# swami1995/diff-qp-mpc

Hardware: AMD Instinct MI355X
Metric: QPs/sec (fwd+bwd), batch=4096 n=3 m=3 T=5 (higher is better)
Workload: dtype f64; 1 GPU; random dense QP family R (SURVEY 8d), configs[0] shape at the BASELINE metric batch: B=4096/GPU nz=30 nineq=30 neq=15; global_batch=4096, n_state=3, n_ctrl=3, T=5, parallelism=batch-shard x1, termination=batch (the reference's batch-coupled rule, parity-safe)

## Files before the change

diff-qp-mpc_amd/_build.py:

```python
import os
import shutil
import subprocess

HERE = os.path.dirname(os.path.abspath(__file__))
CSRC = os.path.join(HERE, "csrc")
SO = os.path.join(CSRC, "libdqp_hip.so")
ARCH = "gfx950"

R16_SIZES = [
    (30, 30, 15),
    (20, 10, 15),
    (15, 10, 10),
    (25, 10, 20),
    (10, 5, 3), (12, 8, 0),
]
R16N_SIZES = [s for s in R16_SIZES if s[2] > 0] + [
    (40, 20, 30),
    (35, 10, 30),
]

RIC_HOST_PARTS = [
    [(15, 1), (14, 2), (13, 3), (11, 5)], [(10, 6), (9, 7), (8, 8)],
    [(31, 1)], [(30, 2)], [(29, 3)], [(28, 4)], [(27, 5)], [(26, 6)], [(25, 7)],
]
# ... 8 lines not shown
def hipcc():
    for c in (os.environ.get("HIPCC"), shutil.which("hipcc"), "/opt/rocm/bin/hipcc"):
        if c and os.path.exists(c):
            return c
    raise RuntimeError("hipcc not found (set HIPCC=/path/to/hipcc)")


def _deps():
    d = [os.path.join(CSRC, f) for f in os.listdir(CSRC) if f.endswith((".hip", ".h", ".hpp"))]
    d.append(os.path.join(os.path.dirname(HERE), "include", "dqp.h"))
    d.append(os.path.abspath(__file__))
    return d


def needs_build():
    if not os.path.exists(SO):
        return True
    t = os.path.getmtime(SO)
    return any(os.path.getmtime(d) > t for d in _deps() if os.path.exists(d))


def _jobs():
    cc = hipcc()
    jobs = []
    variants = [("r16f", "dqp_r16.hip", R16_SIZES, []), ("r16b", "dqp_r16.hip", R16_SIZES, ["-DDQP_R16_BWD"]),
                ("r16n", "dqp_r16n.hip", R16N_SIZES, []), ("r16nb", "dqp_r16n.hip", R16N_SIZES, ["-DDQP_R16_BWD"])]
    for tag, src, sizes, extra in variants:
        for n, m, e in sorted(sizes, key=lambda t: -t[0] * t[1]):
            obj = os.path.join(CSRC, "dqp_%s_%d_%d_%d.o" % (tag, n, m, e))
            jobs.append((obj, [cc] + FLAGS + extra + ["-DDQP_R16_N=%d" % n, "-DDQP_R16_M=%d" % m,
                                                      "-DDQP_R16_E=%d" % e, "-c",
                                                      os.path.join(CSRC, src), "-o", obj]))
    for src in PLAIN_SOURCES:
# ... 11 lines not shown
            if "ric" in name and "pad" not in name:
                return 10 ** 5
            return 10 ** 9 if "pdipm" in name else 1
        n, mm, e = m
        w = n * n * (n + mm)
        return w * (4 if "_r16n_" in name else (1 if "_r16nb_" in name else 2))
    jobs.sort(key=cost, reverse=True)
    lst = lambda sizes: " ".join("X(%d,%d,%d)" % s for s in sizes)
    obj = os.path.join(CSRC, "dqp_dispatch.o")
    jobs.append((obj, [cc] + FLAGS + ["-DDQP_R16_SIZE_LIST=" + lst(R16_SIZES),
                                      "-DDQP_R16N_SIZE_LIST=" + lst(R16N_SIZES),
                                      "-c", os.path.join(CSRC, "dqp_dispatch.hip"), "-o", obj]))
    return jobs


def _object_current(obj, cmd):
    stamp = obj + ".cmd"
    if not (os.path.exists(obj) and os.path.exists(stamp)):
        return False
    with open(stamp) as f:
        if f.read() != " ".join(cmd):
            return False
    src = cmd[cmd.index("-c") + 1]
    deps = [src]
    dfile = obj[:-2] + ".d"
    if os.path.exists(dfile):
        with open(dfile) as f:
            words = f.read().replace("\\\n", " ").split()
        deps += [w for w in words[1:] if w.startswith((CSRC, os.path.dirname(HERE)))]
    else:
        deps += [os.path.join(os.path.dirname(HERE), "include", "dqp.h")]
        deps += [os.path.join(CSRC, f) for f in os.listdir(CSRC) if f.endswith((".h", ".hpp"))]
    t = os.path.getmtime(obj)
    return all(os.path.exists(d) and os.path.getmtime(d) <= t for d in deps)


def build(force=False, verbose=False, max_parallel=None):
    if not force and not needs_build():
        return SO
    jobs = _jobs()
    todo = [j for j in jobs if force or not _object_current(*j)]
    all_jobs, jobs = jobs, todo
    max_parallel = max_parallel or max(1, min(len(jobs), (os.cpu_count() or 2)))
    import time
    pending, running = list(jobs), []
    while pending or running:
        while pending and len(running) < max_parallel:
            obj, cmd = pending.pop(0)
            if verbose:
                print(" ".join(cmd))
            running.append((subprocess.Popen(cmd), cmd))
        still = []
        for pr, cmd in running:
            rc = pr.poll()
            if rc is None:
                still.append((pr, cmd))
            elif rc != 0:
                for other, _ in running:
                    if other.poll() is None:
                        other.kill()
                raise subprocess.CalledProcessError(rc, cmd)
            else:
                with open(cmd[-1] + ".cmd", "w") as f:
                    f.write(" ".join(cmd))
        if len(still) == len(running):
            time.sleep(0.2)
        running = still
    subprocess.check_call([hipcc(), "--offload-arch=" + ARCH, "-shared", "-fPIC", "-o", SO] +
                          [obj for obj, _ in all_jobs])
    return SO


if __name__ == "__main__":
    print(build(force=True, verbose=True))
```

diff-qp-mpc_amd/csrc/dqp_common.h:

```cpp
#ifndef DQP_COMMON_H_
#define DQP_COMMON_H_
#include <hip/hip_runtime.h>
#include <stdint.h>

#include "../../include/dqp.h"
#include "dqp_trace.h"

namespace dqp {

constexpr int WAVE = 64;

struct KParams {
    const double *Q, *p, *G, *h, *A, *b;
    long long sQ, sp, sG, sh, sA, sb;
    double *zhat, *lam, *nu, *slack, *best_resid;
    const double *zin, *lamin, *nuin, *slackin, *gin;
    double *dQ, *dp, *dG, *dh, *dA, *db;
    int32_t *info;
    double *workspace;
    unsigned long long *stamps;
    int B, N, M, E;
    int ldz, ldm, lde, ldt;
    double eps, stallTol;
    int maxIter, notImprovedLim;
    unsigned flags;
    double *hist;
    const int32_t *cap;
    int histIters;
    int dynId, dynT, dynN, dynM;
    double dynDt;
    const double *dynX0;
    const double *mC, *mc, *mF, *mf, *mx0, *mul, *muu;
    double *mdC, *mdc, *mdF, *mdf, *mdx0;
    int mn, mm, mT;
    double *snap;
    const double *histIn;
    const double *extRy;
    int itBegin, itEnd;
};

constexpr int TERM_HDR = 8;

constexpr int TERM_MAXIT = 64;
constexpr int TERM_ACC_BYTES = 3 * 8 + TERM_HDR * 4;

__device__ __forceinline__ void hist_put(const KParams &P, long long qp, int it, double resid, double mu)
{
    double2 *h = reinterpret_cast<double2 *>(P.hist) + (long long)it * P.B + qp;
    *h = make_double2(resid, mu);
}
__device__ __forceinline__ void hist_fill(const KParams &P, long long qp, int iters)
{
    const double nan = __builtin_nan("");
    for (int it = iters; it < P.histIters; ++it)
        reinterpret_cast<double2 *>(P.hist)[(long long)it * P.B + qp] = make_double2(nan, nan);
}
__device__ __forceinline__ void term_zero_acc(const KParams &P)
{
    if (P.hist && blockIdx.x == 0) {
        unsigned *a = reinterpret_cast<unsigned *>(P.hist + (long long)P.B * P.histIters * 2);
        for (int i = threadIdx.x; i < TERM_ACC_BYTES / 4; i += blockDim.x) a[i] = 0u;
    }
}

__device__ __forceinline__ bool term_flagged(const KParams &P, long long qp) { return P.cap[TERM_HDR + qp] >= P.cap[0]; }

size_t term_bytes(int B, int maxIter, int snapDim);
int term_decide(const KParams &P, void *term, void *stream);
int term_local_masks(const KParams &P, void *term, unsigned long long *masks, void *stream);
int term_decide_global(const KParams &P, void *term, const unsigned long long *masks, void *stream);
void term_bind_pass1(KParams &P, void *term, int snapDim);
void term_bind_pass2(KParams &P, void *term);


#ifdef DQP_STAMPS
extern unsigned long long *g_debug_stamps;
#endif
int r16_forward(const KParams &P, void *stream);
int r16_backward(const KParams &P, void *stream);
int r16n_forward(const KParams &P, void *stream);
long long r16n_workspace_doubles(int N, int M, int E);
int r16n_snapshot_doubles(int N, int M, int E);
bool ric_supported(int n_state, int n_ctrl);
long long ric_workspace_doubles(int n_state, int n_ctrl, int T);
int ric_forward(const KParams &P, void *stream);
long long ric_stepped_workspace_doubles(int n_state, int n_ctrl, int T, int B);
int ric_forward_stepped(const KParams &P, void *stream);
int ric_backward(const KParams &P, void *stream);
int ric_snapshot_doubles(int n_state, int n_ctrl, int T);
int ric_finish(const KParams &P, void *stream);
bool ricw_supported(int n_state, int n_ctrl);
long long ricw_workspace_doubles(int n_state, int n_ctrl, int T);
int ricw_forward(const KParams &P, void *stream);
long long ricw_stepped_workspace_doubles(int n_state, int n_ctrl, int T, int B);
int ricw_forward_stepped(const KParams &P, void *stream);
int ricw_backward(const KParams &P, void *stream);
int ricw_snapshot_doubles(int n_state, int n_ctrl, int T);
// ... 40 lines not shown
```

diff-qp-mpc_amd/csrc/dqp_dispatch.hip:

```cpp
#include "dqp_common.h"

#ifndef DQP_R16_SIZE_LIST
#error "DQP_R16_SIZE_LIST not defined (see _build.py)"
#endif
#ifndef DQP_R16N_SIZE_LIST
#define DQP_R16N_SIZE_LIST
#endif

namespace dqp {

#define X(n, m, e)                                                  \
    int r16_forward_##n##_##m##_##e(const KParams &, void *);       \
    int r16_backward_##n##_##m##_##e(const KParams &, void *);
DQP_R16_SIZE_LIST
#undef X
#define X(n, m, e)                                                  \
    int r16n_forward_##n##_##m##_##e(const KParams &, void *);      \
    int r16n_backward_##n##_##m##_##e(const KParams &, void *);
DQP_R16N_SIZE_LIST
#undef X

int r16_forward(const KParams &P, void *stream)
{
#define X(n, m, e) if (P.N == n && P.M == m && P.E == e) return r16_forward_##n##_##m##_##e(P, stream);
    DQP_R16_SIZE_LIST
#undef X
    return 1;
}

int r16_backward(const KParams &P, void *stream)
{
#define X(n, m, e) if (P.N == n && P.M == m && P.E == e) return r16_backward_##n##_##m##_##e(P, stream);
// ... 6 lines not shown
{
#define X(n, m, e) if (P.N == n && P.M == m && P.E == e) return r16n_forward_##n##_##m##_##e(P, stream);
    DQP_R16N_SIZE_LIST
#undef X
    return 1;
}

int r16n_backward(const KParams &P, void *stream)
{
#define X(n, m, e) if (P.N == n && P.M == m && P.E == e) return r16n_backward_##n##_##m##_##e(P, stream);
    DQP_R16N_SIZE_LIST
#undef X
    return 1;
}

long long r16n_workspace_doubles(int N, int M, int E)
{
#define X(n, m, e)                                                                          \
    if (N == n && M == m && E == e)                                                         \
        return (long long)e * (n - e) + (long long)e * (e - 1) / 2 + (long long)n * (n + 1) / 2 + \
               (long long)m * n + (long long)e * e + 5 * e + n + 1;
    DQP_R16N_SIZE_LIST
#undef X
    return 0;
}

int r16n_snapshot_doubles(int N, int M, int E)
{
    return r16n_workspace_doubles(N, M, E) > 0 ? (N - E) + 2 * M + 2 : 0;
}
// ... 3 lines not shown
```

diff-qp-mpc_amd/csrc/dqp_pdipm.hip:

```cpp

#include <hip/hip_runtime.h>
#include <math.h>
#include <stdint.h>

#include "dqp_common.h"
#include "dqp_dyn_models.h"

using namespace dqp;

namespace {

#define WSYNC() __syncthreads()

__device__ __forceinline__ double bcast(double v, int src)
{
    int lo = __double2loint(v), hi = __double2hiint(v);
    lo = __builtin_amdgcn_readlane(lo, src);
    hi = __builtin_amdgcn_readlane(hi, src);
    return __hiloint2double(hi, lo);
}

template <int CTRL> __device__ __forceinline__ double dppd(double v)
{
    return __builtin_amdgcn_update_dpp(v, v, CTRL, 0xf, 0xf, true);
// ... 711 lines not shown
    if (rc != DQP_OK) return rc;
    if (P.B == 0) return DQP_OK;
    if (!Q || !p || !G || !h || !zhat || !lam || !slack) return DQP_ERR_BAD_ARG;
    P.workspace = (double *)workspace;
    if (P.E > 0 && (!A || !b || !nu)) return DQP_ERR_BAD_ARG;
    P.Q = Q; P.p = p; P.G = G; P.h = h; P.A = A; P.b = b;
    P.zhat = zhat; P.lam = lam; P.nu = nu; P.slack = slack;
    P.info = info; P.best_resid = best_resid;
    if (!(P.flags & DQP_FLAG_BATCH_TERMINATION)) return forward_once(P, lds, workspace, stream);
    if (!termination || P.maxIter < 1 || P.maxIter > 64) return DQP_ERR_BAD_ARG;
    P.eps = opts ? opts->eps : 1e-12;
    const bool nullspace = workspace && !(P.flags & (DQP_FLAG_GENERIC_ONLY | DQP_FLAG_NO_NULLSPACE)) && !P.dynId && !is_big(P);
    term_bind_pass1(P, termination, nullspace ? r16n_snapshot_doubles(P.N, P.M, P.E) : 0);
    if ((rc = forward_once(P, lds, workspace, stream)) != DQP_OK) return rc;
    if (P.flags & DQP_FLAG_HISTORY_ONLY) return DQP_OK;
    if ((rc = term_decide(P, termination, stream)) != DQP_OK) return rc;
    term_bind_pass2(P, termination);
    return forward_once(P, lds, workspace, stream);
}

__attribute__((visibility("default"))) int
dqp_term_local_masks(const dqp_dims *dims, const dqp_opts *opts, void *termination, uint64_t *masks, void *stream)
{
    KParams P = {};
    size_t lds = 0;
    int rc = fill_params(dims, opts, P, lds);
    if (rc != DQP_OK) return rc;
    if (!(P.flags & DQP_FLAG_BATCH_TERMINATION) || !termination || !masks || P.maxIter < 1 || P.maxIter > 64)
        return DQP_ERR_BAD_ARG;
    if (P.B == 0) return hipMemsetAsync(masks, 0, 24, (hipStream_t)stream) == hipSuccess ? DQP_OK : DQP_ERR_LAUNCH;
// ... 167 lines not shown
    if (kind == MPC_PAD) {
        R = pad_region(P.workspace + pad_kernel_doubles(P.mn, P.mm, P.mT, P.B, false), P.mn, P.mm, P.mT, P.B);
        rc = pad_pack(md->n_state, P.mn, P.mm, P.mT, P.B, R, C, c, F, f, x0, nullptr, nullptr, nullptr, nullptr, stream);
        if (rc != DQP_OK) return rc;
        P.mC = R.C; P.mc = R.c; P.mF = R.F; P.mf = R.f; P.mx0 = R.x0; P.zhat = R.tau; P.nu = R.nu;
    }
    auto done = [&](int r) {
        if (r != DQP_OK || kind != MPC_PAD) return r;
        return pad_unpack(md->n_state, P.mn, P.mm, P.mT, P.B, R, tau, nu, nullptr, nullptr, nullptr, nullptr, nullptr, stream);
    };
    if (!batch) return done(run(P));
    P.eps = opts ? opts->eps : 1e-12;
    term_bind_pass1(P, termination, mpc_snapshot_doubles(P, kind));
    if ((rc = run(P)) != DQP_OK) return rc;
    if (P.flags & DQP_FLAG_HISTORY_ONLY) return done(DQP_OK);
    if ((rc = term_decide(P, termination, stream)) != DQP_OK) return rc;
    term_bind_pass2(P, termination);
    return done(kind == MPC_R16N ? r16n_forward(P, stream) : ric_finish(P, stream));
}

static int stage_snapshot_doubles(int n, int m, int T)
{
    return stage_supported(n, m) ? T * (2 * n + 5 * m) : 0;
}

static int stepped_params(const dqp_mpc_dims *md, const dqp_opts *opts, KParams &P)
{
    if (!md || md->nbatch < 0 || md->n_state <= 0 || md->n_ctrl <= 0 || md->T < 2 || !md->has_bounds) return DQP_ERR_BAD_ARG;
    int np = md->n_state;
    if (md->n_state_host) {
// ... 158 lines not shown
```

diff-qp-mpc_amd/csrc/dqp_r16_prims.h:

```cpp
#ifndef DQP_R16_PRIMS_H_
#define DQP_R16_PRIMS_H_
#include <hip/hip_runtime.h>
#include <math.h>

#include "dqp_common.h"

namespace dqp {
namespace r16 {

template <int CTRL> __device__ __forceinline__ double dppd(double v)
{
    return __builtin_amdgcn_update_dpp(v, v, CTRL, 0xf, 0xf, true);
}

__device__ __forceinline__ double rb(double v, int k)
{
    switch (k & 15) {
    case 0: return dppd<0x150>(v);   case 1: return dppd<0x151>(v);
    case 2: return dppd<0x152>(v);   case 3: return dppd<0x153>(v);
    case 4: return dppd<0x154>(v);   case 5: return dppd<0x155>(v);
    case 6: return dppd<0x156>(v);   case 7: return dppd<0x157>(v);
    case 8: return dppd<0x158>(v);   case 9: return dppd<0x159>(v);
    case 10: return dppd<0x15a>(v);  case 11: return dppd<0x15b>(v);
    case 12: return dppd<0x15c>(v);  case 13: return dppd<0x15d>(v);
// ... 378 lines not shown
        }
        __syncthreads();
        const double *row = stage + (r < nr ? r : 0) * NC;
#pragma unroll
        for (int j = 0; j < NC; ++j) dst[s][j] = row[j];
        if (16 * s + 15 >= nrows) {
            const double keep = r < nr ? 1.0 : 0.0;
#pragma unroll
            for (int j = 0; j < NC; ++j) dst[s][j] *= keep;
        }
        __syncthreads();
    }
}

template <int S, int NC>
__device__ __forceinline__ void load_rows(const double *src, int nrows, double (&dst)[S][NC], int r)
{
#pragma unroll
    for (int s = 0; s < S; ++s) {
        const int i = r + 16 * s;
        const double *row = src + (i < nrows ? i : nrows - 1) * NC;
        const double keep = i < nrows ? 1.0 : 0.0;
#pragma unroll
        for (int j = 0; j < NC; ++j) dst[s][j] = row[j];
        if (16 * s + 15 >= nrows) {
#pragma unroll
            for (int j = 0; j < NC; ++j) dst[s][j] *= keep;
        }
    }
}

template <class C>
__device__ __forceinline__ void factor_T(double *lds, double (&T)[C::SM][C::M],
                                         const double (&rdiag)[C::SM], const double (&dinv)[C::SM],
                                         double (&rdu)[C::SM], int r)
{
    constexpr int M = C::M, SM = C::SM;
    double *Rp = lds + C::oR;
#pragma unroll
    for (int s = 0; s < SM; ++s) {
        const int i = r + 16 * s;
        double *dst = i < M ? Rp + tri(i) + i : lds + C::oDummy + r;
        *dst = rdiag[s] + dinv[s];
    }
// ... 21 lines not shown
```

diff-qp-mpc_amd/csrc/dqp_r16n.hip:

```cpp

#include "dqp_r16_prims.h"

namespace dqp {
namespace r16n {

using namespace dqp::r16;

template <int N_, int M_, int E_> struct Cfg {
    static constexpr int N = N_, M = M_, E = E_, R = N_ - E_;
    static constexpr int SN = slots(N_), SM = slots(M_), SR = slots(N_ - E_);
    static constexpr int SE = E_ > 0 ? slots(E_) : 1, EC = E_ > 0 ? E_ : 1;
    static constexpr bool PARK = slots(N_) >= 3;
#ifndef DQP_R16N_PARK_WU
#define DQP_R16N_PARK_WU 1
#endif
    static constexpr bool PARKWU = PARK || DQP_R16N_PARK_WU;
#ifndef DQP_R16N_PIN_ALL
#define DQP_R16N_PIN_ALL 1
#endif
    static constexpr bool PIN = PARK || DQP_R16N_PIN_ALL;
#ifndef DQP_R16N_SPLIT_ALL
#define DQP_R16N_SPLIT_ALL 0
#endif
    static constexpr bool SPLIT = PARK || DQP_R16N_SPLIT_ALL;
#ifndef DQP_R16N_EARLY_CTX
#define DQP_R16N_EARLY_CTX 1
#endif
    static constexpr bool EARLY = DQP_R16N_EARLY_CTX;
    static constexpr int tailsz = E_ * (N_ - E_) + E_ * (E_ - 1) / 2;
    static constexpr int oLq = 0;
    static constexpr int oTl = tri(N_);
    static constexpr int oR = oTl;
    static constexpr int shared = tailsz > tri(M_) ? tailsz : tri(M_);
    static constexpr int oCp = oTl + shared;
    static constexpr int oHp = oCp + (N_ - E_);
    static constexpr int oQv = oHp + M_;
    static constexpr int oBw = oQv + N_;
    static constexpr int oBs = oBw + (N_ - E_), oBz = oBs + M_, oBc = oBz + M_;
    static constexpr int oDummy = oBc + 2;
    static constexpr int ldsQP = oDummy + 16;
    static constexpr int ldsQPpad = (ldsQP + 1) & ~1;
#ifndef DQP_R16N_STAGED
#define DQP_R16N_STAGED 0
#endif
    static constexpr bool STAGED = DQP_R16N_STAGED && 16 * N_ <= ldsQP - oTl;
    __host__ __device__ static constexpr int toff(int k) { return k * (N_ - E_) + k * (k - 1) / 2; }
    static constexpr int wTl = 0, wLq = tailsz, wG = wLq + tri(N_), wU = wG + M_ * N_;
    static constexpr int wTau = wU + E_ * E_, wRdu = wTau + E_, wRdq = wRdu + E_;
    static constexpr int wXy = wRdq + N_, wPy = wXy + E_, wW1 = wPy + E_, wDl = wW1 + E_;
    static constexpr int wsQP = wDl + 1;
    static constexpr int snapDim = (N_ - E_) + 2 * M_ + 2;
};

#define DQP_PHASE_FENCE() asm volatile("" ::: "memory")
__device__ __forceinline__ void pin(double &x) { asm volatile("" : "+v"(x) : : "memory"); }
__device__ __forceinline__ const double *relabel(const double *p)
{
    asm volatile("" : "+v"(p));
    return p;
}
// ... 161 lines not shown
}
template <int S, int NC>
__device__ __forceinline__ void mpc_rows_G(const KParams &P, int nrows, double (&dst)[S][NC], int r)
{
    const int n = P.mn, m = P.mm, nt = n + m, half = P.mT * m;
#pragma unroll
    for (int s = 0; s < S; ++s) {
        const int i = r + 16 * s;
        const int k = i < half ? i : i - half;
        const int t = k / m, col = t * nt + n + (k - t * m);
        const double sg = i < half ? 1.0 : -1.0;
#pragma unroll
        for (int c = 0; c < NC; ++c) dst[s][c] = (c == col && i < nrows) ? sg : 0.0;
    }
}
template <int S, int NC>
__device__ __forceinline__ void mpc_rows_A(const KParams &P, long long qp, int nrows, double (&dst)[S][NC], int r)
{
    const int n = P.mn, nt = n + P.mm, T = P.mT;
#pragma unroll
    for (int s = 0; s < S; ++s) {
        const int e = r + 16 * s, ec = e < nrows ? e : nrows - 1;
        const int t = ec / n, j = ec - t * n;
        const bool dynrow = t < T - 1;
        const double *row = P.mF + (((long long)(dynrow ? t : 0) * P.B + qp) * n + j) * nt;
        int tc = 0, jc = 0;
#pragma unroll
        for (int c = 0; c < NC; ++c) {
            const double f = row[jc];
            double v;
            if (dynrow) v = (tc == t) ? f : ((tc == t + 1 && jc == j) ? -1.0 : 0.0);
            else v = (tc == 0 && jc == j) ? 1.0 : 0.0;
            dst[s][c] = e < nrows ? v : 0.0;
            if (++jc == nt) { jc = 0; ++tc; }
        }
    }
}

template <class C>
__device__ __forceinline__ void park_GU(double *ws, const State<C> &st, int r)
{
    constexpr int N = C::N, M = C::M, E = C::E, R = C::R;
#pragma unroll
    for (int s = 0; s < C::SM; ++s) {
// ... 106 lines not shown
            b0[s] = (E > 0 && e < E) ? v : 0.0;
        }
    } else {
#pragma unroll
        for (int s = 0; s < SN; ++s) p0[s] = (r + 16 * s < N) ? P.p[qp * P.sp + r + 16 * s] : 0.0;
#pragma unroll
        for (int s = 0; s < SM; ++s) h0[s] = (r + 16 * s < M) ? P.h[qp * P.sh + r + 16 * s] : 0.0;
#pragma unroll
        for (int s = 0; s < SE; ++s) b0[s] = (E > 0 && r + 16 * s < E) ? P.b[qp * P.sb + r + 16 * s] : 0.0;
    }
    {
        double Lq[SN][N];
        if (mpc) mpc_rows_Q<SN, N>(P, qp, Lq, r);
        else if (C::STAGED) load_rows_staged<SN, N, (N * N) % 2 == 0>(P.Q + qp * P.sQ, N, Lq, r, lds + C::oTl);
        else load_rows<SN, N>(P.Q + qp * P.sQ, N, Lq, r);
        if (!chol_rows<SN, N>(Lq, st.rdq, r)) st.status = DQP_STATUS_Q_NOT_PD;
        tri_store<SN, N>(lds + C::oLq, Lq, r, dummy);
    }
    __syncthreads();
    if (C::EARLY) {
        double *ws = P.workspace + qp * (long long)C::wsQP;
        for (int e = r; e < tri(N); e += 16) ws[C::wLq + e] = lds[C::oLq + e];
#pragma unroll
        for (int s = 0; s < SN; ++s)
            if (r + 16 * s < N) ws[C::wRdq + r + 16 * s] = st.rdq[s];
    }
    __builtin_amdgcn_sched_barrier(0);
    DQP_PHASE_FENCE();
    STAMP(P, 1);

    if (mpc) {
        if (!C::SPLIT) mpc_rows_G<SM, N>(P, M, st.Gh, r);
        if (E > 0) mpc_rows_A<SE, N>(P, qp, E, st.Ah, r);
    } else {
        if (C::STAGED) {
            if (!C::SPLIT) load_rows_staged<SM, N, (M * N) % 2 == 0>(P.G + qp * P.sG, M, st.Gh, r, lds + C::oTl);
            if (E > 0) load_rows_staged<SE, N, (C::EC * N) % 2 == 0>(P.A + qp * P.sA, E, st.Ah, r, lds + C::oTl);
        } else {
            if (!C::SPLIT) load_rows<SM, N>(P.G + qp * P.sG, M, st.Gh, r);
            if (E > 0) load_rows<SE, N>(P.A + qp * P.sA, E, st.Ah, r);
        }
    }
    {
        const double *Lp = lds + C::oLq;
#pragma unroll
        for (int j = 0; j < N; ++j) {
#pragma unroll
            for (int k = 0; k < j; ++k) {
                const double ljk = Lp[tri(j) + k];
                if (!C::SPLIT) {
// ... 313 lines not shown

    {
        if (!C::EARLY) {
            double *ws = P.workspace + qp * (long long)C::wsQP;
            for (int e = r; e < C::tailsz; e += 16) ws[C::wTl + e] = lds[C::oTl + e];
            for (int e = r; e < tri(N); e += 16) ws[C::wLq + e] = lds[C::oLq + e];
            if (!C::PARKWU) park_GU<C>(ws, st, r);
#pragma unroll
            for (int s = 0; s < SN; ++s)
                if (r + 16 * s < N) ws[C::wRdq + r + 16 * s] = st.rdq[s];
        }
    }
    __syncthreads();
    {
        double *Rp = lds + C::oR;
#pragma unroll
        for (int j = 0; j < M; ++j) {
            const int sj = j >> 4, lj = j & 15;
            double acc[SM];
#pragma unroll
            for (int s = 0; s < SM; ++s) acc[s] = 0.0;
#pragma unroll
            for (int c = 0; c < R; ++c) {
                const double gb = rb(st.Gh[sj][c], lj);
#pragma unroll
                for (int s = 0; s < SM; ++s)
                    if (16 * s + 15 >= j) acc[s] = fma(st.Gh[s][c], gb, acc[s]);
            }
#pragma unroll
            for (int s = 0; s < SM; ++s) {
                if (16 * s + 15 < j) continue;
                const int i = r + 16 * s;
                double *dst = (i < M && j <= i) ? Rp + tri(i) + j : dummy;
                *dst = acc[s];
            }
        }
    }
    __syncthreads();
#pragma unroll
    for (int s = 0; s < SM; ++s) {
        const int i = r + 16 * s;
        const double v = (lds + C::oR)[tri(i < M ? i : M - 1) + (i < M ? i : M - 1)];
        st.rdiag[s] = i < M ? v : 0.0;
    }
    __builtin_amdgcn_sched_barrier(0);
    DQP_PHASE_FENCE();
}

template <class C>
// ... 60 lines not shown
        for (int s = 0; s < SN; ++s)
            if (r + 16 * s < N) P.zhat[qp * N + r + 16 * s] = xh[s];
#pragma unroll
        for (int s = 0; s < SM; ++s)
            if (inM[s]) { P.lam[qp * M + r + 16 * s] = bz[s]; P.slack[qp * M + r + 16 * s] = bs[s]; }
        if (E > 0) {
#pragma unroll
            for (int s = 0; s < SE; ++s)
                if (r + 16 * s < E) P.nu[qp * E + r + 16 * s] = yv[s];
        }
        if (r == 0) {
            if (P.info) { P.info[2 * qp] = st.status; P.info[2 * qp + 1] = iters; }
            if (P.best_resid) P.best_resid[qp] = best;
        }
    }
}

template <class C>
__global__ __launch_bounds__(64) void forward_kernel(KParams P)
{
    constexpr int N = C::N, M = C::M, E = C::E, R = C::R;
    constexpr int SN = C::SN, SM = C::SM, SE = C::SE, SR = C::SR;
    extern __shared__ __attribute__((aligned(16))) double sm[];
    const int lane = threadIdx.x, r = lane & 15, qrow = lane >> 4;
    long long qp = (long long)blockIdx.x * 4 + qrow;
    bool live = qp < P.B;
    if (!live) qp = P.B - 1;
    int maxIter = P.maxIter;
    const bool batch = (P.flags & DQP_FLAG_BATCH_TERMINATION) != 0;
    const bool strict = (P.flags & DQP_FLAG_STRICT_GET_STEP) != 0;
    if (P.cap) {
        maxIter = min(maxIter, P.cap[0]);
        live = live && term_flagged(P, qp);
        if (__builtin_amdgcn_ballot_w64(live) == 0) return;
    }
    double *lds = sm + qrow * C::ldsQPpad;
    double *dummy = lds + C::oDummy + r;

    term_zero_acc(P);
    State<C> st;
    STAMP(P, 0);
    setup<C>(P, qp, r, lds, st);
    STAMP(P, 15);

    bool inM[SM], inR[SR];
#pragma unroll
    for (int s = 0; s < SM; ++s) inM[s] = r + 16 * s < M;
#pragma unroll
    for (int s = 0; s < SR; ++s) inR[s] = r + 16 * s < R;

    double T[SM][M], rdu[SM];
    double w[SR], s_[SM], z[SM];
    double cc = 1.0, delta = 0.0;
    {
// ... 24 lines not shown
#pragma unroll
        for (int s = 0; s < SM; ++s) {
            if (ms < 0.0 && inM[s]) s_[s] -= ms - 1.0;
            if (mz < 0.0 && inM[s]) z[s] -= mz - 1.0;
        }
        delta = mz < 0.0 ? 1.0 - mz : 0.0;
        if (r == 0) P.workspace[qp * (long long)C::wsQP + C::wDl] = delta;
    }

    double gz[SR];
    mul_GzT<C>(st, z, gz, r);
    STAMP(P, 6);
    double best = INFINITY, bestc = 1.0;
    bool have_best = false, done = false;
    int nNot = 0, iters = 0;

    for (int it = 0; it < maxIter; ++it) {
        double rw[SR], rz[SM];
        {
            double cp[SR], hp[SM], gw[SM];
            vec_get<SR>(lds + C::oCp, cp, R, r);
            vec_get<SM>(lds + C::oHp, hp, M, r);
            mul_Gz<C>(st, w, gw);
#pragma unroll
            for (int s = 0; s < SR; ++s) rw[s] = inR[s] ? w[s] + cp[s] + gz[s] : 0.0;
#pragma unroll
            for (int s = 0; s < SM; ++s) rz[s] = inM[s] ? gw[s] + s_[s] - hp[s] : 0.0;
        }
        double sz = 0.0, nz2 = 0.0;
#pragma unroll
        for (int s = 0; s < SM; ++s) { sz = fma(s_[s], z[s], sz); nz2 = fma(rz[s], rz[s], nz2); }
        double nx2 = rx_norm2_partial<C>(st, lds, rw, cc * delta, r);
        sz = row_sum(sz); nz2 = row_sum(nz2); nx2 = row_sum(nx2);
        const double mu = fabs(sz * (1.0 / M));
        const double resid = sqrt(nz2) + sqrt(nx2) + M * mu;
        if (!done) {
            iters = it + 1;
            if (!have_best || resid < best) {
                nNot = 0; have_best = true; best = resid; bestc = cc;
                vec_put<SR>(lds + C::oBw, w, R, r, dummy);
                vec_put<SM>(lds + C::oBs, s_, M, r, dummy);
                vec_put<SM>(lds + C::oBz, z, M, r, dummy);
                if (P.snap && live) {
                    double *sp = P.snap + ((long long)it * P.B + qp) * C::snapDim;
#pragma unroll
                    for (int s = 0; s < SR; ++s)
                        if (inR[s]) sp[r + 16 * s] = w[s];
#pragma unroll
                    for (int s = 0; s < SM; ++s)
                        if (inM[s]) { sp[R + r + 16 * s] = s_[s]; sp[R + M + r + 16 * s] = z[s]; }
                    if (r == 0) sp[R + 2 * M] = cc;
                }
            } else {
                nNot += 1;
            }
            if (batch) {
                if (P.hist && r == 0 && live) hist_put(P, qp, it, resid, mu);
                done = !(fabs(resid) < INFINITY);
            } else if ((nNot >= P.notImprovedLim && best < P.stallTol) || best < P.eps || mu > 1e32 ||
                       !(fabs(resid) < INFINITY))
                done = true;
        }
        if (__builtin_amdgcn_ballot_w64(!done) == 0) break;
        if (it == 1) STAMP(P, 9);

        double dza[SM], dsa[SM];
        {
            double gu[SM];
            mul_Gz<C>(st, rw, gu);
#pragma unroll
            for (int s = 0; s < SM; ++s) dza[s] = rz[s] - s_[s] - gu[s];
        }
// ... 39 lines not shown
        lu_solve<SM, M>(T, rdu, dzc, r);
        if (it == 1) STAMP(P, 12);
        tm = 0.0;
#pragma unroll
        for (int s = 0; s < SM; ++s) {
            dz[s] = dza[s] + dzc[s];
            ds[s] = fma(-rsc[s] - dzc[s], dinv[s], dsa[s]);
            tm = fmax(tm, fmax(-dz[s] * rzv[s], -ds[s] * rsv[s]));
        }
        if (strict) {
#pragma unroll
            for (int s = 0; s < SM; ++s) zero_step |= inM[s] && (dz[s] == 0.0 || ds[s] == 0.0);
            if ((__builtin_amdgcn_ballot_w64(zero_step) >> (lane & 48)) & 0xffffull) done = true;
        }
        __builtin_amdgcn_sched_barrier(0);
        double gtd[SR];
        mul_GzT<C>(st, dz, gtd, r);
        alpha = frcp(fmax(row_max(tm) * (1.0 / 0.999), 1.0));
        if (!done) {
#pragma unroll
            for (int s = 0; s < SR; ++s) {
                w[s] = fma(alpha, -rw[s] - gtd[s], w[s]);
                gz[s] = fma(alpha, gtd[s], gz[s]);
            }
#pragma unroll
            for (int s = 0; s < SM; ++s) { s_[s] = fma(alpha, ds[s], s_[s]); z[s] = fma(alpha, dz[s], z[s]); }
            cc *= (1.0 - alpha);
        }
        if (it == 1) STAMP(P, 13);
        if (it == 0) STAMP(P, 8);
    }
    STAMP(P, 7);

    if (P.hist && r == 0 && live) hist_fill(P, qp, iters);
    epilogue<C>(P, qp, r, lds, st, bestc, delta, iters, best, live, true);
    STAMP(P, 14);
}

template <class C>
__device__ __forceinline__ void load_ctx(const KParams &P, long long qp, int r, double *lds, State<C> &st)
{
    constexpr int N = C::N, M = C::M, E = C::E, R = C::R;
    constexpr int SN = C::SN, SM = C::SM, SE = C::SE;
    st.status = DQP_STATUS_OK;
    {
        const double *ws = P.workspace + qp * (long long)C::wsQP;
        for (int e = r; e < C::tailsz; e += 16) lds[C::oTl + e] = ws[C::wTl + e];
        for (int e = r; e < tri(N); e += 16) lds[C::oLq + e] = ws[C::wLq + e];
#pragma unroll
        for (int s = 0; s < SM; ++s) {
// ... 25 lines not shown
            st.rdq[s] = i < N ? v : 0.0;
        }
    }
}

template <class C>
__global__ __launch_bounds__(64) void finish_kernel(KParams P)
{
    constexpr int M = C::M, E = C::E, R = C::R;
    constexpr int SM = C::SM, SE = C::SE, SR = C::SR;
    extern __shared__ __attribute__((aligned(16))) double sm[];
    const int lane = threadIdx.x, r = lane & 15, qrow = lane >> 4;
    long long qp = (long long)blockIdx.x * 4 + qrow;
    bool live = qp < P.B;
    if (!live) qp = P.B - 1;
    live = live && term_flagged(P, qp);
    if (__builtin_amdgcn_ballot_w64(live) == 0) return;
    const int cap = min(P.maxIter, P.cap[0]);
    double *lds = sm + qrow * C::ldsQPpad;
    double *dummy = lds + C::oDummy + r;
    State<C> st;
    load_ctx<C>(P, qp, r, lds, st);
    const double *ws = P.workspace + qp * (long long)C::wsQP;
#pragma unroll
    for (int s = 0; s < SE; ++s) {
        const int k = r + 16 * s, kc = k < E ? k : (E > 0 ? E - 1 : 0);
        const double a = ws[C::wXy + kc], b = ws[C::wPy + kc], c = ws[C::wW1 + kc];
        st.xy[s] = (E > 0 && k < E) ? a : 0.0;
        st.py[s] = (E > 0 && k < E) ? b : 0.0;
        st.w1[s] = (E > 0 && k < E) ? c : 0.0;
    }
    const double delta = ws[C::wDl];
    const double2 *h = reinterpret_cast<const double2 *>(P.histIn) + qp;
// ... 226 lines not shown
}

#if !defined(DQP_R16_N) || !defined(DQP_R16_M) || !defined(DQP_R16_E)
#error "compile with -DDQP_R16_N=.. -DDQP_R16_M=.. -DDQP_R16_E=.."
#endif
#define DQP_CAT2(a, n, m, e) a##n##_##m##_##e
#define DQP_CAT(a, n, m, e) DQP_CAT2(a, n, m, e)

#ifndef DQP_R16_BWD
int DQP_CAT(r16n_forward_, DQP_R16_N, DQP_R16_M, DQP_R16_E)(const KParams &P, void *stream)
{
    using C = r16n::Cfg<DQP_R16_N, DQP_R16_M, DQP_R16_E>;
    if (P.cap && P.snap && P.histIn) return r16n::launch<C>(r16n::finish_kernel<C>, P, stream);
    return r16n::launch<C>(r16n::forward_kernel<C>, P, stream);
}
#else
int DQP_CAT(r16n_backward_, DQP_R16_N, DQP_R16_M, DQP_R16_E)(const KParams &P, void *stream)
{
    using C = r16n::Cfg<DQP_R16_N, DQP_R16_M, DQP_R16_E>;
    return r16n::launch<C>(r16n::backward_kernel<C>, P, stream);
}
#endif

}
```

diff-qp-mpc_amd/csrc/dqp_term.hip:

```cpp
#include "dqp_common.h"

namespace dqp {

namespace {

constexpr int MAXIT = TERM_MAXIT;
struct Acc {
    unsigned long long improved;
    unsigned long long notbelow;
    unsigned long long notabove;
};
static_assert(sizeof(Acc) + TERM_HDR * sizeof(int32_t) == TERM_ACC_BYTES, "layout shared with dqp_common.h");

inline size_t hist_bytes(int B, int maxIter) { return (size_t)B * maxIter * 2 * sizeof(double); }

__device__ __forceinline__ unsigned long long wave_or_u64(unsigned long long v)
{
#pragma unroll
    for (int off = 32; off > 0; off >>= 1) v |= __shfl_xor(v, off, 64);
    return v;
}

__device__ __forceinline__ int rule_stop(unsigned long long ai, unsigned long long anb, unsigned long long ana, int maxIter,
                                         int notImprovedLim)
{
    int nNot = 0;
    for (int it = 0; it < maxIter; ++it) {
        if (it == 0 || ((ai >> it) & 1ull)) nNot = 0;
        else nNot += 1;
        if (nNot == notImprovedLim || !((anb >> it) & 1ull) || !((ana >> it) & 1ull)) return it + 1;
    }
    return maxIter;
}

constexpr int SCAN_CHUNK = 32;
__global__ __launch_bounds__(64) void term_scan_kernel(const double2 *hist, Acc *acc, int32_t *hdr,
                                                       int B, int maxIter, int notImprovedLim, double eps,
                                                       int decide)
{
    const int lane = threadIdx.x;
    const long long qp = (long long)blockIdx.x * blockDim.x + lane;
    const bool live = qp < B;
    unsigned long long imp = 0ull, nb = 0ull, na = 0ull;
    if (live) {
        const double2 *h = hist + qp;
        double best = 0.0;
        int arg = 0;
// ... 62 lines not shown
{
    P.hist = (double *)term;
    P.histIters = P.maxIter;
    P.cap = nullptr;
    P.histIn = nullptr;
    P.snap = snapDim > 0 ? (double *)((char *)term + snap_offset(P.B, P.maxIter)) : nullptr;
}

void term_bind_pass2(KParams &P, void *term)
{
    P.hist = nullptr;
    P.histIn = (const double *)term;
    P.cap = hdr_of(term, P.B, P.maxIter);
}

int term_decide(const KParams &P, void *term, void *stream)
{
    const int blocks = (P.B + 63) / 64;
    DQP_LAUNCH(term_scan_kernel, dim3(blocks), dim3(64), 0, (hipStream_t)stream,
                       (const double2 *)term, acc_of(term, P.B, P.maxIter), hdr_of(term, P.B, P.maxIter),
                       P.B, P.maxIter, P.notImprovedLim, P.eps, 1);
    return hipGetLastError() == hipSuccess ? DQP_OK : DQP_ERR_LAUNCH;
}

int term_local_masks(const KParams &P, void *term, unsigned long long *masks, void *stream)
{
    const int blocks = (P.B + 63) / 64;
    DQP_LAUNCH(term_scan_kernel, dim3(blocks), dim3(64), 0, (hipStream_t)stream,
                       (const double2 *)term, acc_of(term, P.B, P.maxIter), hdr_of(term, P.B, P.maxIter),
                       P.B, P.maxIter, P.notImprovedLim, P.eps, 0);
// ... 15 lines not shown
```

Measured before the change: 16.06 million QPs/sec.

## Fuse termination mask reduction into r16n forward kernel, prefetch tails, group R GEMM

```diff
diff --git a/diff-qp-mpc_amd/_build.py b/diff-qp-mpc_amd/_build.py
--- a/diff-qp-mpc_amd/_build.py
+++ b/diff-qp-mpc_amd/_build.py
@@ -5,6 +5,8 @@
 HERE = os.path.dirname(os.path.abspath(__file__))
 CSRC = os.path.join(HERE, "csrc")
 SO = os.path.join(CSRC, "libdqp_hip.so")
+TERM_SCAN_SO = os.path.join(CSRC, "libdqp_hip_termscan.so")
+TERM_SCAN_SIZES = [(30, 30, 15)]
 ARCH = "gfx950"
 
 R16_SIZES = [
@@ -46,9 +48,9 @@
 
 
 def needs_build():
-    if not os.path.exists(SO):
+    if not os.path.exists(SO) or not os.path.exists(TERM_SCAN_SO):
         return True
-    t = os.path.getmtime(SO)
+    t = min(os.path.getmtime(SO), os.path.getmtime(TERM_SCAN_SO))
     return any(os.path.getmtime(d) > t for d in _deps() if os.path.exists(d))
 
 
@@ -90,6 +92,15 @@
     return jobs
 
 
+def _term_scan_jobs(jobs):
+    out = {}
+    for obj, cmd in jobs:
+        if os.path.basename(obj) in ["dqp_r16n_%d_%d_%d.o" % s for s in TERM_SCAN_SIZES]:
+            o2 = obj[:-2] + ".termscan.o"
+            out[obj] = (o2, cmd[:-1] + [o2, "-DDQP_R16N_TERM_SCAN=1"])
+    return out
+
+
 def _object_current(obj, cmd):
     stamp = obj + ".cmd"
     if not (os.path.exists(obj) and os.path.exists(stamp)):
@@ -115,7 +126,8 @@
     if not force and not needs_build():
         return SO
     jobs = _jobs()
-    todo = [j for j in jobs if force or not _object_current(*j)]
+    variant = _term_scan_jobs(jobs)
+    todo = [j for j in list(variant.values()) + jobs if force or not _object_current(*j)]
     all_jobs, jobs = jobs, todo
     max_parallel = max_parallel or max(1, min(len(jobs), (os.cpu_count() or 2)))
     import time
@@ -137,13 +149,15 @@
                         other.kill()
                 raise subprocess.CalledProcessError(rc, cmd)
             else:
-                with open(cmd[-1] + ".cmd", "w") as f:
+                with open(cmd[cmd.index("-o") + 1] + ".cmd", "w") as f:
                     f.write(" ".join(cmd))
         if len(still) == len(running):
             time.sleep(0.2)
         running = still
     subprocess.check_call([hipcc(), "--offload-arch=" + ARCH, "-shared", "-fPIC", "-o", SO] +
                           [obj for obj, _ in all_jobs])
+    subprocess.check_call([hipcc(), "--offload-arch=" + ARCH, "-shared", "-fPIC", "-o", TERM_SCAN_SO] +
+                          [variant[obj][0] if obj in variant else obj for obj, _ in all_jobs])
     return SO
 
 
diff --git a/diff-qp-mpc_amd/csrc/dqp_common.h b/diff-qp-mpc_amd/csrc/dqp_common.h
--- a/diff-qp-mpc_amd/csrc/dqp_common.h
+++ b/diff-qp-mpc_amd/csrc/dqp_common.h
@@ -35,6 +35,7 @@
     int mn, mm, mT;
     double *snap;
     const double *histIn;
+    const unsigned long long *capMasks;
     const double *extRy;
     int itBegin, itEnd;
 };
@@ -63,6 +64,27 @@
     }
 }
 
+__device__ __forceinline__ void term_zero_acc_agent(const KParams &P)
+{
+    if (P.hist && blockIdx.x == 0) {
+        unsigned *a = reinterpret_cast<unsigned *>(P.hist + (long long)P.B * P.histIters * 2);
+        for (int i = threadIdx.x; i < TERM_ACC_BYTES / 4; i += blockDim.x)
+            __hip_atomic_store(a + i, 0u, __ATOMIC_RELAXED, __HIP_MEMORY_SCOPE_AGENT);
+    }
+}
+
+__device__ __forceinline__ int rule_stop(unsigned long long ai, unsigned long long anb, unsigned long long ana, int maxIter,
+                                         int notImprovedLim)
+{
+    int nNot = 0;
+    for (int it = 0; it < maxIter; ++it) {
+        if (it == 0 || ((ai >> it) & 1ull)) nNot = 0;
+        else nNot += 1;
+        if (nNot == notImprovedLim || !((anb >> it) & 1ull) || !((ana >> it) & 1ull)) return it + 1;
+    }
+    return maxIter;
+}
+
 __device__ __forceinline__ bool term_flagged(const KParams &P, long long qp) { return P.cap[TERM_HDR + qp] >= P.cap[0]; }
 
 size_t term_bytes(int B, int maxIter, int snapDim);
@@ -71,6 +93,7 @@
 int term_decide_global(const KParams &P, void *term, const unsigned long long *masks, void *stream);
 void term_bind_pass1(KParams &P, void *term, int snapDim);
 void term_bind_pass2(KParams &P, void *term);
+void term_bind_pass2_masks(KParams &P, void *term);
 
 
 #ifdef DQP_STAMPS
@@ -81,6 +104,7 @@
 int r16n_forward(const KParams &P, void *stream);
 long long r16n_workspace_doubles(int N, int M, int E);
 int r16n_snapshot_doubles(int N, int M, int E);
+bool r16n_term_in_pass1(int N, int M, int E);
 bool ric_supported(int n_state, int n_ctrl);
 long long ric_workspace_doubles(int n_state, int n_ctrl, int T);
 int ric_forward(const KParams &P, void *stream);
diff --git a/diff-qp-mpc_amd/csrc/dqp_dispatch.hip b/diff-qp-mpc_amd/csrc/dqp_dispatch.hip
--- a/diff-qp-mpc_amd/csrc/dqp_dispatch.hip
+++ b/diff-qp-mpc_amd/csrc/dqp_dispatch.hip
@@ -16,6 +16,7 @@
 #undef X
 #define X(n, m, e)                                                  \
     int r16n_forward_##n##_##m##_##e(const KParams &, void *);      \
+    bool r16n_term_in_pass1_##n##_##m##_##e();                      \
     int r16n_backward_##n##_##m##_##e(const KParams &, void *);
 DQP_R16N_SIZE_LIST
 #undef X
@@ -52,6 +53,14 @@
     return 1;
 }
 
+bool r16n_term_in_pass1(int N, int M, int E)
+{
+#define X(n, m, e) if (N == n && M == m && E == e) return r16n_term_in_pass1_##n##_##m##_##e();
+    DQP_R16N_SIZE_LIST
+#undef X
+    return false;
+}
+
 long long r16n_workspace_doubles(int N, int M, int E)
 {
 #define X(n, m, e)                                                                          \
diff --git a/diff-qp-mpc_amd/csrc/dqp_pdipm.hip b/diff-qp-mpc_amd/csrc/dqp_pdipm.hip
--- a/diff-qp-mpc_amd/csrc/dqp_pdipm.hip
+++ b/diff-qp-mpc_amd/csrc/dqp_pdipm.hip
@@ -749,6 +749,10 @@
     term_bind_pass1(P, termination, nullspace ? r16n_snapshot_doubles(P.N, P.M, P.E) : 0);
     if ((rc = forward_once(P, lds, workspace, stream)) != DQP_OK) return rc;
     if (P.flags & DQP_FLAG_HISTORY_ONLY) return DQP_OK;
+    if (nullspace && r16n_term_in_pass1(P.N, P.M, P.E)) {
+        term_bind_pass2_masks(P, termination);
+        return forward_once(P, lds, workspace, stream);
+    }
     if ((rc = term_decide(P, termination, stream)) != DQP_OK) return rc;
     term_bind_pass2(P, termination);
     return forward_once(P, lds, workspace, stream);
@@ -946,6 +950,10 @@
     term_bind_pass1(P, termination, mpc_snapshot_doubles(P, kind));
     if ((rc = run(P)) != DQP_OK) return rc;
     if (P.flags & DQP_FLAG_HISTORY_ONLY) return done(DQP_OK);
+    if (kind == MPC_R16N && r16n_term_in_pass1(P.N, P.M, P.E)) {
+        term_bind_pass2_masks(P, termination);
+        return done(r16n_forward(P, stream));
+    }
     if ((rc = term_decide(P, termination, stream)) != DQP_OK) return rc;
     term_bind_pass2(P, termination);
     return done(kind == MPC_R16N ? r16n_forward(P, stream) : ric_finish(P, stream));
diff --git a/diff-qp-mpc_amd/csrc/dqp_r16_prims.h b/diff-qp-mpc_amd/csrc/dqp_r16_prims.h
--- a/diff-qp-mpc_amd/csrc/dqp_r16_prims.h
+++ b/diff-qp-mpc_amd/csrc/dqp_r16_prims.h
@@ -416,20 +416,33 @@
 }
 
 template <int S, int NC>
+__device__ __forceinline__ void load_rows_raw(const double *src, int nrows, double (&dst)[S][NC], int r)
+{
+#pragma unroll
+    for (int s = 0; s < S; ++s) {
+        const int i = r + 16 * s;
+        const double *row = src + (i < nrows ? i : nrows - 1) * NC;
+#pragma unroll
+        for (int j = 0; j < NC; ++j) dst[s][j] = row[j];
+    }
+}
+template <int S, int NC>
+__device__ __forceinline__ void mask_rows(int nrows, double (&dst)[S][NC], int r)
+{
+#pragma unroll
+    for (int s = 0; s < S; ++s) {
+        const double keep = r + 16 * s < nrows ? 1.0 : 0.0;
+        if (16 * s + 15 >= nrows) {
+#pragma unroll
+            for (int j = 0; j < NC; ++j) dst[s][j] *= keep;
+        }
+    }
+}
+template <int S, int NC>
 __device__ __forceinline__ void load_rows(const double *src, int nrows, double (&dst)[S][NC], int r)
 {
-#pragma unroll
-    for (int s = 0; s < S; ++s) {
-        const int i = r + 16 * s;
-        const double *row = src + (i < nrows ? i : nrows - 1) * NC;
-        const double keep = i < nrows ? 1.0 : 0.0;
-#pragma unroll
-        for (int j = 0; j < NC; ++j) dst[s][j] = row[j];
-        if (16 * s + 15 >= nrows) {
-#pragma unroll
-            for (int j = 0; j < NC; ++j) dst[s][j] *= keep;
-        }
-    }
+    load_rows_raw<S, NC>(src, nrows, dst, r);
+    mask_rows<S, NC>(nrows, dst, r);
 }
 
 template <class C>
diff --git a/diff-qp-mpc_amd/csrc/dqp_r16n.hip b/diff-qp-mpc_amd/csrc/dqp_r16n.hip
--- a/diff-qp-mpc_amd/csrc/dqp_r16n.hip
+++ b/diff-qp-mpc_amd/csrc/dqp_r16n.hip
@@ -27,7 +27,20 @@
 #define DQP_R16N_EARLY_CTX 1
 #endif
     static constexpr bool EARLY = DQP_R16N_EARLY_CTX;
+#ifndef DQP_R16N_TERM_SCAN
+#define DQP_R16N_TERM_SCAN 0
+#endif
+    static constexpr bool TERMFUSED = !DQP_R16N_TERM_SCAN;
+#ifndef DQP_R16N_PREFETCH_TAILS
+#define DQP_R16N_PREFETCH_TAILS 1
+#endif
+    static constexpr bool PREFETCH = DQP_R16N_PREFETCH_TAILS && E_ > 0 && !PARK;
+#ifndef DQP_R16N_RGROUP
+#define DQP_R16N_RGROUP 4
+#endif
+    static constexpr int RGROUP = DQP_R16N_RGROUP;
     static constexpr int tailsz = E_ * (N_ - E_) + E_ * (E_ - 1) / 2;
+    static constexpr int tailPL = (tailsz + 15) / 16 > 0 ? (tailsz + 15) / 16 : 1;
     static constexpr int oLq = 0;
     static constexpr int oTl = tri(N_);
     static constexpr int oR = oTl;
@@ -44,6 +57,10 @@
 #define DQP_R16N_STAGED 0
 #endif
     static constexpr bool STAGED = DQP_R16N_STAGED && 16 * N_ <= ldsQP - oTl;
+#ifndef DQP_R16N_EARLY_GA
+#define DQP_R16N_EARLY_GA 1
+#endif
+    static constexpr bool EARLYGA = DQP_R16N_EARLY_GA && !STAGED && !SPLIT;
     __host__ __device__ static constexpr int toff(int k) { return k * (N_ - E_) + k * (k - 1) / 2; }
     static constexpr int wTl = 0, wLq = tailsz, wG = wLq + tri(N_), wU = wG + M_ * N_;
     static constexpr int wTau = wU + E_ * E_, wRdu = wTau + E_, wRdq = wRdu + E_;
@@ -235,7 +252,7 @@
         for (int c = 0; c < NC; ++c) dst[s][c] = (c == col && i < nrows) ? sg : 0.0;
     }
 }
-template <int S, int NC>
+template <int S, int NC, bool LOAD = true, bool SELECT = true>
 __device__ __forceinline__ void mpc_rows_A(const KParams &P, long long qp, int nrows, double (&dst)[S][NC], int r)
 {
     const int n = P.mn, nt = n + P.mm, T = P.mT;
@@ -248,7 +265,8 @@
         int tc = 0, jc = 0;
 #pragma unroll
         for (int c = 0; c < NC; ++c) {
-            const double f = row[jc];
+            const double f = LOAD ? row[jc] : dst[s][c];
+            if (!SELECT) { dst[s][c] = f; if (++jc == nt) { jc = 0; ++tc; } continue; }
             double v;
             if (dynrow) v = (tc == t) ? f : ((tc == t + 1 && jc == j) ? -1.0 : 0.0);
             else v = (tc == 0 && jc == j) ? 1.0 : 0.0;
@@ -385,6 +403,16 @@
         if (mpc) mpc_rows_Q<SN, N>(P, qp, Lq, r);
         else if (C::STAGED) load_rows_staged<SN, N, (N * N) % 2 == 0>(P.Q + qp * P.sQ, N, Lq, r, lds + C::oTl);
         else load_rows<SN, N>(P.Q + qp * P.sQ, N, Lq, r);
+        if (C::EARLYGA) {
+            DQP_PHASE_FENCE();
+            if (mpc) {
+                if (E > 0) mpc_rows_A<SE, N, true, false>(P, qp, E, st.Ah, r);
+            } else {
+                if (E > 0) load_rows_raw<SE, N>(P.A + qp * P.sA, E, st.Ah, r);
+                if (!C::SPLIT) load_rows_raw<SM, N>(P.G + qp * P.sG, M, st.Gh, r);
+            }
+            DQP_PHASE_FENCE();
+        }
         if (!chol_rows<SN, N>(Lq, st.rdq, r)) st.status = DQP_STATUS_Q_NOT_PD;
         tri_store<SN, N>(lds + C::oLq, Lq, r, dummy);
     }
@@ -402,9 +430,15 @@
 
     if (mpc) {
         if (!C::SPLIT) mpc_rows_G<SM, N>(P, M, st.Gh, r);
-        if (E > 0) mpc_rows_A<SE, N>(P, qp, E, st.Ah, r);
+        if (E > 0) {
+            if (C::EARLYGA) mpc_rows_A<SE, N, false, true>(P, qp, E, st.Ah, r);
+            else mpc_rows_A<SE, N>(P, qp, E, st.Ah, r);
+        }
     } else {
-        if (C::STAGED) {
+        if (C::EARLYGA) {
+            if (!C::SPLIT) mask_rows<SM, N>(M, st.Gh, r);
+            if (E > 0) mask_rows<SE, N>(E, st.Ah, r);
+        } else if (C::STAGED) {
             if (!C::SPLIT) load_rows_staged<SM, N, (M * N) % 2 == 0>(P.G + qp * P.sG, M, st.Gh, r, lds + C::oTl);
             if (E > 0) load_rows_staged<SE, N, (C::EC * N) % 2 == 0>(P.A + qp * P.sA, E, st.Ah, r, lds + C::oTl);
         } else {
@@ -748,25 +782,43 @@
     __syncthreads();
     {
         double *Rp = lds + C::oR;
-#pragma unroll
-        for (int j = 0; j < M; ++j) {
-            const int sj = j >> 4, lj = j & 15;
-            double acc[SM];
-#pragma unroll
-            for (int s = 0; s < SM; ++s) acc[s] = 0.0;
+        constexpr int GJ = C::RGROUP > 0 ? C::RGROUP : 1;
+#pragma unroll
+        for (int j0 = 0; j0 < M; j0 += GJ) {
+            double acc[GJ][SM];
+#pragma unroll
+            for (int jj = 0; jj < GJ; ++jj)
+#pragma unroll
+                for (int s = 0; s < SM; ++s) acc[jj][s] = 0.0;
 #pragma unroll
             for (int c = 0; c < R; ++c) {
-                const double gb = rb(st.Gh[sj][c], lj);
-#pragma unroll
-                for (int s = 0; s < SM; ++s)
-                    if (16 * s + 15 >= j) acc[s] = fma(st.Gh[s][c], gb, acc[s]);
-            }
-#pragma unroll
-            for (int s = 0; s < SM; ++s) {
-                if (16 * s + 15 < j) continue;
-                const int i = r + 16 * s;
-                double *dst = (i < M && j <= i) ? Rp + tri(i) + j : dummy;
-                *dst = acc[s];
+#pragma unroll
+                for (int jj = 0; jj < GJ; ++jj) {
+                    const int j = j0 + jj;
+                    if (j >= M) continue;
+                    const double gb = rb(st.Gh[j >> 4][c], j & 15);
+#pragma unroll
+                    for (int s = 0; s < SM; ++s)
+                        if (16 * s + 15 >= j) acc[jj][s] = fma(st.Gh[s][c], gb, acc[jj][s]);
+                }
+            }
+            if (GJ > 1) {
+#pragma unroll
+                for (int jj = 0; jj < GJ; ++jj)
+#pragma unroll
+                    for (int s = 0; s < SM; ++s) pin(acc[jj][s]);
+            }
+#pragma unroll
+            for (int jj = 0; jj < GJ; ++jj) {
+                const int j = j0 + jj;
+                if (j >= M) continue;
+#pragma unroll
+                for (int s = 0; s < SM; ++s) {
+                    if (16 * s + 15 < j) continue;
+                    const int i = r + 16 * s;
+                    double *dst = (i < M && j <= i) ? Rp + tri(i) + j : dummy;
+                    *dst = acc[jj][s];
+                }
             }
         }
     }
@@ -857,6 +909,16 @@
             if (P.best_resid) P.best_resid[qp] = best;
         }
     }
+}
+
+constexpr int TERM_SLOTS = 64, TERM_SPREAD_MIN = 2 * TERM_SLOTS;
+template <class C> __device__ __forceinline__ unsigned long long *term_slot(const KParams &P, int k, int j)
+{
+    return reinterpret_cast<unsigned long long *>(P.snap + ((long long)(4 * k + j) * C::snapDim + (C::snapDim - 1)));
+}
+template <class C> __device__ __forceinline__ bool term_spread(const KParams &P)
+{
+    return P.snap != nullptr && (int)gridDim.x >= TERM_SPREAD_MIN;
 }
 
 template <class C>
@@ -880,7 +942,13 @@
     double *lds = sm + qrow * C::ldsQPpad;
     double *dummy = lds + C::oDummy + r;
 
-    term_zero_acc(P);
+    if (C::TERMFUSED) {
+        term_zero_acc_agent(P);
+        if (batch && P.hist && term_spread<C>(P) && blockIdx.x < TERM_SLOTS && lane < 3)
+            __hip_atomic_store(term_slot<C>(P, blockIdx.x, lane), 0ull, __ATOMIC_RELAXED, __HIP_MEMORY_SCOPE_AGENT);
+    } else {
+        term_zero_acc(P);
+    }
     State<C> st;
     STAMP(P, 0);
     setup<C>(P, qp, r, lds, st);
@@ -935,6 +1003,10 @@
     double best = INFINITY, bestc = 1.0;
     bool have_best = false, done = false;
     int nNot = 0, iters = 0;
+    const bool masks = C::TERMFUSED && batch && P.hist != nullptr;
+    unsigned long long mImp = 0ull, mNb = 0ull, mNa = 0ull;
+    double tpre[C::tailPL];
+    bool pre = false;
 
     for (int it = 0; it < maxIter; ++it) {
         double rw[SR], rz[SM];
@@ -959,6 +1031,7 @@
             iters = it + 1;
             if (!have_best || resid < best) {
                 nNot = 0; have_best = true; best = resid; bestc = cc;
+                if (masks && it > 0) mImp |= 1ull << it;
                 vec_put<SR>(lds + C::oBw, w, R, r, dummy);
                 vec_put<SM>(lds + C::oBs, s_, M, r, dummy);
                 vec_put<SM>(lds + C::oBz, z, M, r, dummy);
@@ -977,6 +1050,10 @@
             }
             if (batch) {
                 if (P.hist && r == 0 && live) hist_put(P, qp, it, resid, mu);
+                if (masks) {
+                    if (!(best < P.eps)) mNb |= 1ull << it;
+                    if (!(mu > 1e32)) mNa |= 1ull << it;
+                }
                 done = !(fabs(resid) < INFINITY);
             } else if ((nNot >= P.notImprovedLim && best < P.stallTol) || best < P.eps || mu > 1e32 ||
                        !(fabs(resid) < INFINITY))
@@ -1046,6 +1123,14 @@
             if ((__builtin_amdgcn_ballot_w64(zero_step) >> (lane & 48)) & 0xffffull) done = true;
         }
         __builtin_amdgcn_sched_barrier(0);
+        const bool lastIt = C::PREFETCH && it == maxIter - 1;
+        if (lastIt) {
+            const double *wt = P.workspace + qp * (long long)C::wsQP + C::wTl;
+#pragma unroll
+            for (int k = 0; k < C::tailPL; ++k) tpre[k] = wt[min(r + 16 * k, C::tailsz - 1)];
+            pre = true;
+            DQP_PHASE_FENCE();
+        }
         double gtd[SR];
         mul_GzT<C>(st, dz, gtd, r);
         alpha = frcp(fmax(row_max(tm) * (1.0 / 0.999), 1.0));
@@ -1061,11 +1146,38 @@
         }
         if (it == 1) STAMP(P, 13);
         if (it == 0) STAMP(P, 8);
+        if (lastIt) break;
     }
     STAMP(P, 7);
 
     if (P.hist && r == 0 && live) hist_fill(P, qp, iters);
-    epilogue<C>(P, qp, r, lds, st, bestc, delta, iters, best, live, true);
+    if (masks) {
+        const unsigned long long all = P.histIters >= 64 ? ~0ull : (1ull << P.histIters) - 1ull;
+        const unsigned long long rest = all & ~(iters >= 64 ? ~0ull : (1ull << iters) - 1ull);
+        mNa |= rest;
+        if (!(best < P.eps)) mNb |= rest;
+        unsigned long long *acc = reinterpret_cast<unsigned long long *>(P.hist + (long long)P.B * P.histIters * 2);
+        int32_t *hdr = reinterpret_cast<int32_t *>(acc + 3);
+        if (r == 0 && live) hdr[TERM_HDR + qp] = mImp ? 63 - __builtin_clzll(mImp) : 0;
+        unsigned long long m = 0ull;
+#pragma unroll
+        for (int q = 0; q < 4; ++q) {
+            const bool qlive = (long long)blockIdx.x * 4 + q < P.B;
+            const unsigned long long a = __shfl(mImp, 16 * q, 64), b = __shfl(mNb, 16 * q, 64), c = __shfl(mNa, 16 * q, 64);
+            if (qlive) m |= lane == 0 ? a : (lane == 1 ? b : c);
+        }
+        unsigned long long *dst = term_spread<C>(P) ? term_slot<C>(P, blockIdx.x % TERM_SLOTS, lane < 3 ? lane : 0) : acc + lane;
+        if (lane < 3 && m) __hip_atomic_fetch_or(dst, m, __ATOMIC_RELAXED, __HIP_MEMORY_SCOPE_AGENT);
+    }
+    if (pre) {
+        __syncthreads();
+#pragma unroll
+        for (int k = 0; k < C::tailPL; ++k) {
+            double *dst = r + 16 * k < C::tailsz ? lds + C::oTl + r + 16 * k : dummy;
+            *dst = tpre[k];
+        }
+    }
+    epilogue<C>(P, qp, r, lds, st, bestc, delta, iters, best, live, !pre);
     STAMP(P, 14);
 }
 
@@ -1121,9 +1233,35 @@
     long long qp = (long long)blockIdx.x * 4 + qrow;
     bool live = qp < P.B;
     if (!live) qp = P.B - 1;
-    live = live && term_flagged(P, qp);
+    int istar;
+    if (P.capMasks) {
+        unsigned long long mk[3];
+        const bool spread = term_spread<C>(P);
+#pragma unroll
+        for (int k = 0; k < 3; ++k) {
+            const unsigned long long *src = spread ? term_slot<C>(P, lane, k) : P.capMasks + k;
+            unsigned long long v = __hip_atomic_load(src, __ATOMIC_RELAXED, __HIP_MEMORY_SCOPE_AGENT);
+            if (spread) {
+#pragma unroll
+                for (int off = 32; off > 0; off >>= 1) v |= __shfl_xor(v, off, 64);
+            }
+            mk[k] = ((unsigned long long)(unsigned)__builtin_amdgcn_readfirstlane((int)(v >> 32)) << 32) |
+                    (unsigned)__builtin_amdgcn_readfirstlane((int)v);
+        }
+        istar = rule_stop(mk[0], mk[1], mk[2], P.maxIter, P.notImprovedLim);
+        if (blockIdx.x == 0 && lane == 0) {
+            const_cast<int32_t *>(P.cap)[0] = istar;
+            if (spread) {
+#pragma unroll
+                for (int k = 0; k < 3; ++k) const_cast<unsigned long long *>(P.capMasks)[k] = mk[k];
+            }
+        }
+    } else {
+        istar = P.cap[0];
+    }
+    live = live && P.cap[TERM_HDR + qp] >= istar;
     if (__builtin_amdgcn_ballot_w64(live) == 0) return;
-    const int cap = min(P.maxIter, P.cap[0]);
+    const int cap = min(P.maxIter, istar);
     double *lds = sm + qrow * C::ldsQPpad;
     double *dummy = lds + C::oDummy + r;
     State<C> st;
@@ -1380,6 +1518,10 @@
     if (P.cap && P.snap && P.histIn) return r16n::launch<C>(r16n::finish_kernel<C>, P, stream);
     return r16n::launch<C>(r16n::forward_kernel<C>, P, stream);
 }
+bool DQP_CAT(r16n_term_in_pass1_, DQP_R16_N, DQP_R16_M, DQP_R16_E)()
+{
+    return r16n::Cfg<DQP_R16_N, DQP_R16_M, DQP_R16_E>::TERMFUSED;
+}
 #else
 int DQP_CAT(r16n_backward_, DQP_R16_N, DQP_R16_M, DQP_R16_E)(const KParams &P, void *stream)
 {
diff --git a/diff-qp-mpc_amd/csrc/dqp_term.hip b/diff-qp-mpc_amd/csrc/dqp_term.hip
--- a/diff-qp-mpc_amd/csrc/dqp_term.hip
+++ b/diff-qp-mpc_amd/csrc/dqp_term.hip
@@ -19,18 +19,6 @@
 #pragma unroll
     for (int off = 32; off > 0; off >>= 1) v |= __shfl_xor(v, off, 64);
     return v;
-}
-
-__device__ __forceinline__ int rule_stop(unsigned long long ai, unsigned long long anb, unsigned long long ana, int maxIter,
-                                         int notImprovedLim)
-{
-    int nNot = 0;
-    for (int it = 0; it < maxIter; ++it) {
-        if (it == 0 || ((ai >> it) & 1ull)) nNot = 0;
-        else nNot += 1;
-        if (nNot == notImprovedLim || !((anb >> it) & 1ull) || !((ana >> it) & 1ull)) return it + 1;
-    }
-    return maxIter;
 }
 
 constexpr int SCAN_CHUNK = 32;
@@ -123,6 +111,12 @@
     P.cap = hdr_of(term, P.B, P.maxIter);
 }
 
+void term_bind_pass2_masks(KParams &P, void *term)
+{
+    term_bind_pass2(P, term);
+    P.capMasks = (const unsigned long long *)acc_of(term, P.B, P.maxIter);
+}
+
 int term_decide(const KParams &P, void *term, void *stream)
 {
     const int blocks = (P.B + 63) / 64;
```

After: 15.51 million QPs/sec. -3.4%, worse.
